# enoche/MMRec

Hardware: AMD Instinct MI355X
Metric: GCN-layer edges/sec (3-layer user-item CSR SpMM, d=64, fp32) (higher is better)
Workload: dtype f32

## Files before the change

### include/mmrec_hip.h

```cpp
#ifndef MMREC_HIP_H
#define MMREC_HIP_H

#include <stddef.h>
#include <stdint.h>

#ifdef __cplusplus
extern "C" {
#endif

#define MMREC_ABI_VERSION 16
#define MMREC_EMB_DIM 64

#define MMREC_ERR_BAD_ARG 10001
#define MMREC_ERR_UNSUPPORTED 10002

typedef void* mmrec_stream_t;

int mmrec_abi_version(void);
const char* mmrec_error_string(int err);

#ifndef MMREC_SPMM_CHUNK
#define MMREC_SPMM_CHUNK 512
#endif
#define MMREC_SPMM_LONG_ROW_DEFAULT 32

int mmrec_spmm_csr_f32(const int32_t* rowptr, const int32_t* colidx, const float* vals,
                       const float* X, float* Y, const float* Z, const float* acc_in, float* acc_out,
                       int32_t n_rows, int32_t d, float alpha, float beta, float acc_scale,
                       int32_t long_row_threshold, const int32_t* long_rows,
                       const int32_t* long_chunk_ptr, int32_t n_long, int32_t n_chunks,
                       float* partials, int32_t* long_tickets, mmrec_stream_t stream);

int mmrec_spmm_rows_f32(const int32_t* rowptr, const int32_t* colidx, const float* vals, const float* X,
                        const float* Z, int32_t z_compact, const int64_t* rows, int32_t n_list, int32_t d,
                        int32_t long_row_threshold, float* Y, mmrec_stream_t stream);
int mmrec_spmm_rows_any_f32(const int32_t* rowptr, const int32_t* colidx, const float* vals, const float* X,
                            const float* Z, int32_t z_compact, const int64_t* rows, int32_t n_list, int32_t d,
                            int32_t long_row_threshold, int32_t max_row_chunks, float* Y, mmrec_stream_t stream);
int mmrec_spmm_push_rows_f32(const int32_t* rowptr, const int32_t* colidx, const float* vals, const float* G,
                             float g_scale, const int64_t* rows, int32_t n_list, int32_t d, float* dX, float* dZ,
                             mmrec_stream_t stream);

int mmrec_spmm_csr_f32_layergcn(const int32_t* rowptr, const int32_t* colidx, const float* vals, const float* X,
                                float* Y, const float* ego, float* scaled, float* w, const float* acc_in,
                                float* acc_out, int32_t n_rows, int32_t d, int32_t long_row_threshold,
                                const int32_t* long_rows, const int32_t* long_chunk_ptr, int32_t n_long,
                                int32_t n_chunks, float* partials, int32_t* long_tickets, mmrec_stream_t stream);
int mmrec_spmm_plan_count(const int32_t* rowptr_host, int32_t n_rows, int32_t long_row_threshold,
                          int32_t* n_long, int32_t* n_chunks);
int mmrec_spmm_plan_fill(const int32_t* rowptr_host, int32_t n_rows, int32_t long_row_threshold,
                         int32_t* long_rows, int32_t* long_chunk_ptr);

int mmrec_cos_scale_fwd_f32(const float* E, const float* Ego, float* Out, float* w, float* acc,
                            int32_t n_rows, int32_t d, mmrec_stream_t stream);
int mmrec_cos_scale_bwd_f32(const float* dOut, const float* E, const float* Ego, const float* w,
                            float* dE, float* dEgo_accum, int32_t n_rows, int32_t d,
                            mmrec_stream_t stream);

#define MMREC_BPR_LOGSIG 0
#define MMREC_BPR_GAMMA 1

size_t mmrec_bpr_workspace_bytes(int32_t batch);
int mmrec_bpr_fwd_f32(const float* U, const float* P, const float* N, const int64_t* users,
                      const int64_t* pos, const int64_t* neg, int32_t batch, int32_t d,
                      int32_t variant, float scale, float* loss_out, float* coef, void* workspace,
                      mmrec_stream_t stream);
int mmrec_bpr_bwd_f32(const float* U, const float* P, const float* N, const int64_t* users,
                      const int64_t* pos, const int64_t* neg, int32_t batch, int32_t d,
                      const float* coef, const float* grad_scalar, float scale, float* dU, float* dP,
                      float* dN, mmrec_stream_t stream);
// ... 202 lines not shown
```

### mmrec_amd/_lib.py

```python
from __future__ import annotations

import ctypes
import os
from ctypes import c_char_p, c_float, c_int32, c_int64, c_size_t, c_uint64, c_void_p

import torch

_PKG = os.path.dirname(os.path.abspath(__file__))
LIB_PATH = os.environ.get("MMREC_HIP_LIB") or os.path.join(_PKG, "lib", "libmmrec_hip.so")
ABI_VERSION = 16

_P = c_void_p

SIGNATURES = {
    "mmrec_abi_version": (c_int32, []),
    "mmrec_error_string": (c_char_p, [c_int32]),
    "mmrec_spmm_csr_f32": (c_int32, [_P, _P, _P, _P, _P, _P, _P, _P, c_int32, c_int32, c_float,
                                     c_float, c_float, c_int32, _P, _P, c_int32, c_int32, _P, _P, _P]),
    "mmrec_spmm_csr_f32_layergcn": (c_int32, [_P, _P, _P, _P, _P, _P, _P, _P, _P, _P, c_int32, c_int32, c_int32,
                                              _P, _P, c_int32, c_int32, _P, _P, _P]),
    "mmrec_spmm_plan_count": (c_int32, [_P, c_int32, c_int32, _P, _P]),
    "mmrec_spmm_plan_fill": (c_int32, [_P, c_int32, c_int32, _P, _P]),
    "mmrec_cos_scale_fwd_f32": (c_int32, [_P, _P, _P, _P, _P, c_int32, c_int32, _P]),
    "mmrec_cos_scale_bwd_f32": (c_int32, [_P, _P, _P, _P, _P, _P, c_int32, c_int32, _P]),
    "mmrec_bpr_workspace_bytes": (c_size_t, [c_int32]),
    "mmrec_bpr_fwd_f32": (c_int32, [_P, _P, _P, _P, _P, _P, c_int32, c_int32, c_int32, c_float, _P,
                                    _P, _P, _P]),
    "mmrec_spmm_rows_f32": (c_int32, [_P, _P, _P, _P, _P, c_int32, _P, c_int32, c_int32, c_int32, _P, _P]),
    "mmrec_spmm_rows_any_f32": (c_int32, [_P, _P, _P, _P, _P, c_int32, _P, c_int32, c_int32, c_int32, c_int32, _P, _P]),
    "mmrec_spmm_push_rows_f32": (c_int32, [_P, _P, _P, _P, c_float, _P, c_int32, c_int32, _P, _P, _P]),
    "mmrec_bpr_dots_f32": (c_int32, [_P, _P, _P, _P, _P, _P, c_int32, c_int32, _P, _P]),
    "mmrec_bpr_loss_from_dots_f32": (c_int32, [_P, c_int32, c_int32, c_float, _P, _P, _P, _P]),
    "mmrec_bpr_bwd_f32": (c_int32, [_P, _P, _P, _P, _P, _P, c_int32, c_int32, _P, _P, c_float, _P, _P,
                                    _P, _P]),
    "mmrec_gather_sqnorm_fwd_f32": (c_int32, [_P, _P, c_int32, c_int32, _P, _P, _P]),
    "mmrec_gather_scale_add_bwd_f32": (c_int32, [_P, _P, c_int32, c_int32, _P, _P, _P]),
    "mmrec_infonce_workspace_bytes": (c_size_t, [c_int32]),
    "mmrec_infonce_fwd_f32": (c_int32, [_P, _P, _P, c_int32, c_int32, c_float, _P, _P, _P]),
    "mmrec_infonce_bwd_f32": (c_int32, [_P, c_int32, c_int32, c_float, _P, _P, _P, _P, _P]),
    "mmrec_linear_workspace_bytes": (c_size_t, [c_int32, c_int32, c_int32]),
    "mmrec_linear_fwd_f32": (c_int32, [_P, _P, _P, _P, c_int32, c_int32, c_int32, _P, _P]),
    "mmrec_linear_fwd_split_f32": (c_int32, [_P, _P, _P, _P, c_int32, c_int32, c_int32, _P, _P]),
    "mmrec_linear_bwd_split_workspace_bytes": (c_size_t, [c_int32, c_int32, c_int32]),
# ... 107 lines not shown
```

### mmrec_amd/csrc/spmm.hip

```cpp
#include "common.h"
#include "spmm_narrow.h"

#ifndef MMREC_SPMM_RPG
#define MMREC_SPMM_RPG(n_rows) ((n_rows) <= (1 << 18) ? 1 : 4)
#endif

namespace {

__device__ __forceinline__ void st_coherent(float4* p, float4 v) {
    unsigned long long* q = reinterpret_cast<unsigned long long*>(p);
    const unsigned long long lo = ((unsigned long long)__float_as_uint(v.y) << 32) | __float_as_uint(v.x);
    const unsigned long long hi = ((unsigned long long)__float_as_uint(v.w) << 32) | __float_as_uint(v.z);
    __hip_atomic_store(q, lo, __ATOMIC_RELAXED, __HIP_MEMORY_SCOPE_AGENT);
    __hip_atomic_store(q + 1, hi, __ATOMIC_RELAXED, __HIP_MEMORY_SCOPE_AGENT);
}
__device__ __forceinline__ float4 ld_coherent(const float4* p) {
    unsigned long long* q = reinterpret_cast<unsigned long long*>(const_cast<float4*>(p));
    const unsigned long long lo = __hip_atomic_load(q, __ATOMIC_RELAXED, __HIP_MEMORY_SCOPE_AGENT);
    const unsigned long long hi = __hip_atomic_load(q + 1, __ATOMIC_RELAXED, __HIP_MEMORY_SCOPE_AGENT);
    return make_float4(__uint_as_float((unsigned)lo), __uint_as_float((unsigned)(lo >> 32)),
                       __uint_as_float((unsigned)hi), __uint_as_float((unsigned)(hi >> 32)));
}

struct RowEpilogue {
    const float* Z;
    float* Y;
    const float* acc_in;
    float* acc_out;
    float alpha, beta, acc_scale;
    const float* ego;
    float* scaled;
    float* w_out;
};

template <int DCH, bool LG>
__device__ __forceinline__ void store_row(const RowEpilogue& ep, int row, int lane16, const float4 (&sum)[DCH]) {
    if (DCH == 1 && LG) {
        const size_t off = (size_t)row * 16 + lane16;
        const float4 y = f4_scale(ep.alpha, sum[0]);
        const float4 g = reinterpret_cast<const float4*>(ep.ego)[off];
        const float dot = row16_sum(f4_dot(y, g));
        const float ne = fmaxf(sqrtf(row16_sum(f4_dot(y, y))), 1e-8f);
        const float ng = fmaxf(sqrtf(row16_sum(f4_dot(g, g))), 1e-8f);
        const float w = dot / (ne * ng);
        const float4 o = f4_scale(w, y);
        if (ep.Y) reinterpret_cast<float4*>(ep.Y)[off] = y;
        reinterpret_cast<float4*>(ep.scaled)[off] = o;
        if (lane16 == 0) ep.w_out[row] = w;
        if (ep.acc_out)
            reinterpret_cast<float4*>(ep.acc_out)[off] =
                ep.acc_in ? f4_add(reinterpret_cast<const float4*>(ep.acc_in)[off], o) : o;
        return;
    }
#pragma unroll
    for (int ch = 0; ch < DCH; ++ch) {
// ... 49 lines not shown
    const int lane16 = threadIdx.x & 15, g = threadIdx.x >> 4;
#pragma unroll
    for (int ch = 0; ch < DCH; ++ch) {
        float4 t = f4_zero();
        for (int c = c0 + g; c < c1; c += 16) {
            const float4* src = reinterpret_cast<const float4*>(partials) + (size_t)c * (16 * DCH) + ch * 16 + lane16;
            t = f4_add(t, COHERENT ? ld_coherent(src) : *src);
        }
        red[g][ch * 16 + lane16] = t;
    }
    __syncthreads();
    if (g == 0) {
        float4 r[DCH];
#pragma unroll
        for (int ch = 0; ch < DCH; ++ch) {
            r[ch] = red[0][ch * 16 + lane16];
#pragma unroll
            for (int k = 1; k < 16; ++k) r[ch] = f4_add(r[ch], red[k][ch * 16 + lane16]);
        }
        store_row<DCH, LG>(ep, row, lane16, r);
    }
}

template <int DCH, bool LG>
__global__ __launch_bounds__(256) void spmm_rows_kernel(
    const int32_t* __restrict__ rowptr, const int32_t* __restrict__ colidx,
    const float* __restrict__ vals, const float* __restrict__ X, RowEpilogue ep, int n_rows,
    int long_t, int rows_per_group, const int32_t* __restrict__ long_rows,
    const int32_t* __restrict__ long_chunk_ptr, int n_long, int n_chunks,
    float* __restrict__ partials, int32_t* __restrict__ tickets) {
    __shared__ float4 red[16][16 * DCH];
    __shared__ int s_last;
    const int lane16 = threadIdx.x & 15;
    const int g = threadIdx.x >> 4;
    const float4* X4 = reinterpret_cast<const float4*>(X);
    if ((int)blockIdx.x < n_chunks) {
        const int chunk = blockIdx.x;
        int lo = 0, hi = n_long;
        while (hi - lo > 1) {
            const int mid = (lo + hi) >> 1;
            if (long_chunk_ptr[mid] <= chunk) lo = mid; else hi = mid;
        }
        const int row = long_rows[lo];
        const int cs = rowptr[row] + (chunk - long_chunk_ptr[lo]) * MMREC_SPMM_CHUNK;
        const int ce = min(cs + MMREC_SPMM_CHUNK, rowptr[row + 1]);
        float4 acc[DCH];
#pragma unroll
        for (int ch = 0; ch < DCH; ++ch) acc[ch] = f4_zero();
        for (int base = cs + g * 16; base < ce; base += 256)
            gather_span<DCH>(colidx, vals, X4, base, min(base + 16, ce), lane16, acc);
#pragma unroll
        for (int ch = 0; ch < DCH; ++ch) red[g][ch * 16 + lane16] = acc[ch];
        __syncthreads();
// ... 12 lines not shown
                for (int ch = 0; ch < DCH; ++ch) {
                    float4* dst = reinterpret_cast<float4*>(partials) + (size_t)chunk * (16 * DCH) + ch * 16 + lane16;
                    if (tickets) st_coherent(dst, t[ch]); else *dst = t[ch];
                }
            }
        }
        const int c0 = long_chunk_ptr[lo], c1 = long_chunk_ptr[lo + 1];
        if (!tickets || c1 - c0 == 1) return;
        if (threadIdx.x < 64) {
            __atomic_signal_fence(__ATOMIC_SEQ_CST);
            __builtin_amdgcn_s_waitcnt(0);
            __atomic_signal_fence(__ATOMIC_SEQ_CST);
            __builtin_amdgcn_fence(__ATOMIC_RELEASE, "workgroup");
            if (threadIdx.x == 0)
                s_last = __hip_atomic_fetch_add(tickets + lo, 1, __ATOMIC_RELAXED, __HIP_MEMORY_SCOPE_AGENT) == c1 - c0 - 1;
        }
        __syncthreads();
        if (!s_last) return;
        __builtin_amdgcn_fence(__ATOMIC_ACQUIRE, "workgroup");
        reduce_long_row<DCH, true, LG>(partials, c0, c1, row, ep, red);
        if (threadIdx.x == 0) __hip_atomic_store(tickets + lo, 0, __ATOMIC_RELAXED, __HIP_MEMORY_SCOPE_AGENT);
        return;
    }
    const int row0 = ((int)blockIdx.x - n_chunks) * 16 * rows_per_group + g;
#pragma unroll 1
    for (int i = 0; i < rows_per_group; ++i) {
        const int row = row0 + i * 16;
        if (row >= n_rows) break;
        const int s = rowptr[row], e = rowptr[row + 1];
        if (e - s > long_t) continue;
        float4 acc[DCH];
#pragma unroll
        for (int ch = 0; ch < DCH; ++ch) acc[ch] = f4_zero();
        gather_span<DCH>(colidx, vals, X4, s, e, lane16, acc);
        store_row<DCH, LG>(ep, row, lane16, acc);
    }
}

template <int DCH, bool LG>
__global__ __launch_bounds__(256) void spmm_long_reduce_kernel(
    const int32_t* __restrict__ long_rows, const int32_t* __restrict__ long_chunk_ptr, int n_long,
    const float* __restrict__ partials, RowEpilogue ep) {
    __shared__ float4 red[16][16 * DCH];
    const int i = blockIdx.x;
    const int c0 = long_chunk_ptr[i], c1 = long_chunk_ptr[i + 1];
    if (c1 - c0 <= 1) return;
    reduce_long_row<DCH, false, LG>(partials, c0, c1, long_rows[i], ep, red);
}

template <int DCH, bool LG = false>
void launch_spmm(hipStream_t s, int blocks, int nch, const int32_t* rowptr, const int32_t* colidx,
                 const float* vals, const float* X, const RowEpilogue& ep, int n_rows, int long_t,
                 int rows_per_group, const int32_t* long_rows, const int32_t* long_chunk_ptr, int n_long,
                 float* partials, int32_t* tickets) {
    hipLaunchKernelGGL((spmm_rows_kernel<DCH, LG>), dim3(blocks + nch), dim3(256), 0, s, rowptr, colidx, vals, X,
                       ep, n_rows, long_t, rows_per_group, long_rows, long_chunk_ptr, n_long, nch, partials, tickets);
    if (!tickets && n_long > 0 && nch > n_long)
        hipLaunchKernelGGL((spmm_long_reduce_kernel<DCH, LG>), dim3(n_long), dim3(256), 0, s, long_rows,
                           long_chunk_ptr, n_long, partials, ep);
}

__global__ __launch_bounds__(256) void cos_scale_fwd_kernel(const float* __restrict__ E,
                                                            const float* __restrict__ Ego,
                                                            float* __restrict__ Out,
                                                            float* __restrict__ W,
                                                            float* __restrict__ acc, int n_rows) {
    const int lane16 = threadIdx.x & 15;
    const int row = blockIdx.x * 16 + (threadIdx.x >> 4);
    if (row >= n_rows) return;
    const size_t off = (size_t)row * 16 + lane16;
    const float4 e = reinterpret_cast<const float4*>(E)[off];
    const float4 g = reinterpret_cast<const float4*>(Ego)[off];
    const float dot = row16_sum(f4_dot(e, g));
    const float ne = fmaxf(sqrtf(row16_sum(f4_dot(e, e))), 1e-8f);
    const float ng = fmaxf(sqrtf(row16_sum(f4_dot(g, g))), 1e-8f);
    const float w = dot / (ne * ng);
    const float4 o = f4_scale(w, e);
    reinterpret_cast<float4*>(Out)[off] = o;
    if (lane16 == 0) W[row] = w;
// ... 8 lines not shown
    if (row >= n_rows) return;
    const size_t off = (size_t)row * 16 + lane16;
    const float4 e = reinterpret_cast<const float4*>(E)[off];
    const float4 g = reinterpret_cast<const float4*>(Ego)[off];
    const float4 d = reinterpret_cast<const float4*>(dOut)[off];
    const float w = W[row];
    const float ne_raw = sqrtf(row16_sum(f4_dot(e, e)));
    const float ng_raw = sqrtf(row16_sum(f4_dot(g, g)));
    const float ne = fmaxf(ne_raw, 1e-8f), ng = fmaxf(ng_raw, 1e-8f);
    const float dw = row16_sum(f4_dot(d, e));
    const float inv = 1.0f / (ne * ng);
    const float ce = (ne_raw > 1e-8f) ? w / (ne * ne) : 0.f;
    const float cg = (ng_raw > 1e-8f) ? w / (ng * ng) : 0.f;
    float4 de = f4_scale(w, d);
    de = f4_fma(dw * inv, g, de);
    de = f4_fma(-dw * ce, e, de);
    reinterpret_cast<float4*>(dE)[off] = de;
    float4 dg = reinterpret_cast<float4*>(dEgo)[off];
    dg = f4_fma(dw * inv, e, dg);
    dg = f4_fma(-dw * cg, g, dg);
    reinterpret_cast<float4*>(dEgo)[off] = dg;
}

}

extern "C" int mmrec_spmm_csr_f32(const int32_t* rowptr, const int32_t* colidx, const float* vals,
                                  const float* X, float* Y, const float* Z, const float* acc_in,
                                  float* acc_out, int32_t n_rows, int32_t d, float alpha, float beta,
                                  float acc_scale, int32_t long_row_threshold,
                                  const int32_t* long_rows, const int32_t* long_chunk_ptr,
                                  int32_t n_long, int32_t n_chunks, float* partials, int32_t* long_tickets,
                                  mmrec_stream_t stream) {
    const bool narrow = d == 8 || d == 16 || d == 32;
    if (!narrow && (d <= 0 || d % MMREC_EMB_DIM || d / MMREC_EMB_DIM > 6)) return MMREC_ERR_UNSUPPORTED;
    if (n_rows < 0 || n_long < 0 || n_chunks < 0 || long_row_threshold < 0) return MMREC_ERR_BAD_ARG;
    if (n_rows == 0) return 0;
    if (!rowptr || !X || (!Y && !acc_out)) return MMREC_ERR_BAD_ARG;
    if (acc_out && !acc_in) return MMREC_ERR_BAD_ARG;
    if (n_long > 0 && (!long_rows || !long_chunk_ptr || !partials || n_chunks <= 0))
        return MMREC_ERR_BAD_ARG;
    if (Y == X || acc_out == X) return MMREC_ERR_BAD_ARG;
    if (narrow)
        return spmm_narrow_launch(rowptr, colidx, vals, X, Y, Z, acc_in, acc_out, n_rows, d, alpha, beta, acc_scale,
                                  n_long > 0 ? long_row_threshold : INT32_MAX, long_rows, long_chunk_ptr, n_long,
                                  n_long > 0 ? n_chunks : 0, partials, mmrec_stream(stream));
    RowEpilogue ep{Z, Y, acc_in, acc_out, alpha, Z ? beta : 0.f, acc_scale, nullptr, nullptr, nullptr};
// ... 51 lines not shown
                                           const float* X, float* Y, const float* ego, float* scaled, float* w,
                                           const float* acc_in, float* acc_out, int32_t n_rows, int32_t d,
                                           int32_t long_row_threshold, const int32_t* long_rows,
                                           const int32_t* long_chunk_ptr, int32_t n_long, int32_t n_chunks,
                                           float* partials, int32_t* long_tickets, mmrec_stream_t stream) {
    if (d != MMREC_EMB_DIM) return MMREC_ERR_UNSUPPORTED;
    if (n_rows < 0 || n_long < 0 || n_chunks < 0 || long_row_threshold < 0) return MMREC_ERR_BAD_ARG;
    if (n_rows == 0) return 0;
    if (!rowptr || !X || !ego || !scaled || !w) return MMREC_ERR_BAD_ARG;
    if (n_long > 0 && (!long_rows || !long_chunk_ptr || !partials || n_chunks <= 0)) return MMREC_ERR_BAD_ARG;
    if (Y == X || scaled == X || acc_out == X) return MMREC_ERR_BAD_ARG;
    RowEpilogue ep{nullptr, Y, acc_in, acc_out, 1.f, 0.f, 1.f, ego, scaled, w};
    hipStream_t s = mmrec_stream(stream);
    const int rows_per_group = MMREC_SPMM_RPG(n_rows);
    const int blocks = (n_rows + 16 * rows_per_group - 1) / (16 * rows_per_group);
    const int long_t = n_long > 0 ? long_row_threshold : INT32_MAX;
    const int nch = n_long > 0 ? n_chunks : 0;
    int32_t* tickets = n_long > 0 ? long_tickets : nullptr;
    launch_spmm<1, true>(s, blocks, nch, rowptr, colidx, vals, X, ep, n_rows, long_t, rows_per_group, long_rows,
                         long_chunk_ptr, n_long, partials, tickets);
    MMREC_RETURN_LAUNCH_STATUS();
}

extern "C" int mmrec_spmm_plan_count(const int32_t* rowptr_host, int32_t n_rows,
                                     int32_t long_row_threshold, int32_t* n_long, int32_t* n_chunks) {
    if (!rowptr_host || !n_long || !n_chunks || n_rows < 0) return MMREC_ERR_BAD_ARG;
    int32_t nl = 0, nc = 0;
    for (int32_t r = 0; r < n_rows; ++r) {
        const int32_t deg = rowptr_host[r + 1] - rowptr_host[r];
        if (deg > long_row_threshold) {
            ++nl;
            nc += (deg + MMREC_SPMM_CHUNK - 1) / MMREC_SPMM_CHUNK;
        }
    }
    *n_long = nl;
    *n_chunks = nc;
    return 0;
}

extern "C" int mmrec_spmm_plan_fill(const int32_t* rowptr_host, int32_t n_rows,
                                    int32_t long_row_threshold, int32_t* long_rows,
                                    int32_t* long_chunk_ptr) {
    if (!rowptr_host || !long_rows || !long_chunk_ptr || n_rows < 0) return MMREC_ERR_BAD_ARG;
    int32_t nl = 0, nc = 0;
    for (int32_t r = 0; r < n_rows; ++r) {
        const int32_t deg = rowptr_host[r + 1] - rowptr_host[r];
// ... 33 lines not shown
```

### mmrec_amd/hip_ops.py

```python
from __future__ import annotations

import ctypes

import numpy as np
import torch

from . import _lib

EMB_DIM = 64
LINEAR_F16X3_DEFAULT = True
LINEAR_F16X3 = LINEAR_F16X3_DEFAULT
SLICE_WIDTHS = (8, 16, 32)
SPMM_CHUNK = 512
LONG_ROW_DEFAULT = None


def default_long_row_threshold(n_cols):
    import os
    forced = os.environ.get("MMREC_LONG_ROW_THRESHOLD")
    if forced:
        return int(forced)
    return 16 if n_cols <= (1 << 18) else 32

TOPK_MAX = 128
BPR_LOGSIG, BPR_GAMMA = 0, 1

DETERMINISTIC_DEFAULT = False
DETERMINISTIC = DETERMINISTIC_DEFAULT
_TORCH_DET_BY_US = False


def set_deterministic(flag=True):
    global DETERMINISTIC, _TORCH_DET_BY_US
    DETERMINISTIC = bool(flag)
    if DETERMINISTIC and not torch.are_deterministic_algorithms_enabled():
        torch.use_deterministic_algorithms(True, warn_only=True)
        _TORCH_DET_BY_US = True
    elif not DETERMINISTIC and _TORCH_DET_BY_US:
        torch.use_deterministic_algorithms(False)
        _TORCH_DET_BY_US = False


def scatter_add_rows(ids, rows, out):
    lib = _lib.load()
    _chk(ids, torch.int64, "ids", 1)
# ... 11 lines not shown
def _stream():
    return ctypes.c_void_p(torch.cuda.current_stream().cuda_stream)


def _chk(t, dtype, name, dim=None):
    if not isinstance(t, torch.Tensor) or not t.is_cuda:
        raise _lib.MMRecHipError("%s must be a device tensor (the hot path has no CPU fallback)" % name)
    if t.dtype != dtype:
        raise _lib.MMRecHipError("%s must be %s, got %s" % (name, dtype, t.dtype))
    if not t.is_contiguous():
        raise _lib.MMRecHipError("%s must be contiguous" % name)
    if dim is not None and t.dim() != dim:
        raise _lib.MMRecHipError("%s must be %d-d" % (name, dim))
    return t


def _ws(nbytes, device):
    return torch.empty(max(int(nbytes), 16), dtype=torch.uint8, device=device)


class CsrGraph:

    def __init__(self, rowptr, colidx, vals, n_rows, n_cols, symmetric=False,
                 long_row_threshold=LONG_ROW_DEFAULT, rowptr_host=None):
        self.rowptr = _chk(rowptr, torch.int32, "rowptr", 1)
        self.colidx = _chk(colidx, torch.int32, "colidx", 1)
        self.vals = _chk(vals, torch.float32, "vals", 1)
        self.n_rows, self.n_cols = int(n_rows), int(n_cols)
        self.nnz = int(colidx.numel())
        self.symmetric = bool(symmetric)
        self.long_row_threshold = int(default_long_row_threshold(self.n_cols) if long_row_threshold is None
                                      else long_row_threshold)
        self._t = self if symmetric else None
        self._plan(rowptr_host)

    def _plan(self, rowptr_host):
        lib = _lib.load()
        rp = rowptr_host if rowptr_host is not None else self.rowptr.cpu().numpy()
        rp = np.ascontiguousarray(rp, dtype=np.int32)
        self.rowptr_host = rp
        n_long, n_chunks = ctypes.c_int32(0), ctypes.c_int32(0)
        _lib.check(lib.mmrec_spmm_plan_count(rp.ctypes.data_as(ctypes.c_void_p), self.n_rows,
                                             self.long_row_threshold, ctypes.byref(n_long),
                                             ctypes.byref(n_chunks)), "spmm_plan_count")
        self.n_long, self.n_chunks = n_long.value, n_chunks.value
        dev = self.rowptr.device
        if self.n_long > 0:
            lr = np.empty(self.n_long, dtype=np.int32)
            cp = np.empty(self.n_long + 1, dtype=np.int32)
            _lib.check(lib.mmrec_spmm_plan_fill(rp.ctypes.data_as(ctypes.c_void_p), self.n_rows,
                                                self.long_row_threshold,
                                                lr.ctypes.data_as(ctypes.c_void_p),
                                                cp.ctypes.data_as(ctypes.c_void_p)), "spmm_plan_fill")
            self.long_rows = torch.from_numpy(lr).to(dev)
            self.long_chunk_ptr = torch.from_numpy(cp).to(dev)
            self.max_row_chunks = int(np.diff(cp).max())
            self.long_tickets = torch.zeros(self.n_long, dtype=torch.int32, device=dev)
        else:
            self.long_rows = self.long_chunk_ptr = self.long_tickets = None
            self.max_row_chunks = 1
        self._partials = {}

    def checked(self, rc, what):
        try:
            _lib.check(rc, what)
        except _lib.MMRecHipError:
            if self.long_tickets is not None:
                try:
                    self.long_tickets.zero_()
                except RuntimeError:
                    pass
            raise

    def partials_for(self, d):
        if self.n_long == 0:
            return None
        if d not in self._partials:
            self._partials[d] = torch.empty(self.n_chunks * d, dtype=torch.float32, device=self.rowptr.device)
        return self._partials[d]

    @classmethod
    def from_coo_host(cls, idx, val, n_rows, n_cols, device, symmetric=False, **kw):
        idx = np.asarray(idx, dtype=np.int64)
        val = np.asarray(val, dtype=np.float32)
# ... 21 lines not shown
        return cls(rowptr, colidx, vout, n_rows, n_cols, symmetric=symmetric, **kw)

    def to_coo_host(self):
        rp = self.rowptr_host.astype(np.int64)
        rows = np.repeat(np.arange(self.n_rows, dtype=np.int64), np.diff(rp))
        return np.stack([rows, self.colidx.cpu().numpy().astype(np.int64)]), self.vals.cpu().numpy()

    def transpose(self):
        if self._t is None:
            idx, val = self.to_coo_host()
            self._t = CsrGraph.from_coo_host(idx[::-1], val, self.n_cols, self.n_rows,
                                             self.rowptr.device,
                                             long_row_threshold=self.long_row_threshold)
            self._t._t = self
        return self._t

    def row_block(self, r0, r1):
        rp = self.rowptr_host.astype(np.int64)
        s, e = int(rp[r0]), int(rp[r1])
        rph = (rp[r0:r1 + 1] - s).astype(np.int32)
        dev = self.rowptr.device
        return CsrGraph(torch.from_numpy(rph).to(dev), self.colidx[s:e].contiguous(),
                        self.vals[s:e].contiguous(), r1 - r0, self.n_cols,
                        long_row_threshold=self.long_row_threshold, rowptr_host=rph)


def _mode_labels(rows, lab_c, n_rows, n_labels):
    key = rows.astype(np.int64) * n_labels + lab_c
    key.sort()
    start = np.flatnonzero(np.concatenate([[True], key[1:] != key[:-1]]))
    cnt = np.diff(np.concatenate([start, [key.shape[0]]]))
    k = key[start]
    r, lab = k // n_labels, k % n_labels
    o = np.lexsort((lab, -cnt, r))
    r_s = r[o]
    first = np.concatenate([[True], r_s[1:] != r_s[:-1]])
    out = np.full(n_rows, -1, dtype=np.int64)
    out[r_s[first]] = lab[o][first]
    return out


def _mode_labels_device(rows, lab_c, n_rows, n_labels):
    key, _ = torch.sort(rows * n_labels + lab_c)
    uk, cnt = torch.unique_consecutive(key, return_counts=True)
    r, lab = torch.div(uk, n_labels, rounding_mode='floor'), uk % n_labels
    cmax = int(cnt.max().item()) + 1
    if n_rows * cmax * n_labels >= 2 ** 62:
# ... 64 lines not shown
        self.n_rows = self.n_cols = n
        self.nnz = g.nnz

    def to_new(self, X):
        return X.index_select(0, self.inv)

    def to_old(self, Xp):
        return Xp.index_select(0, self.perm)


def spmm_raw(g: CsrGraph, X, Y=None, Z=None, acc_in=None, acc_out=None, alpha=1.0, beta=1.0,
             acc_scale=1.0):
    lib = _lib.load()
    _chk(X, torch.float32, "X", 2)
    d = X.shape[1]
    if (d not in SLICE_WIDTHS and (d % EMB_DIM or d > 6 * EMB_DIM)) or X.shape[0] < g.n_cols:
        raise _lib.MMRecHipError("X must be [>=%d, 64*k <= 384 (or a feature slice of 8 / 16 / 32 columns)], got %s" %
                                 (g.n_cols, tuple(X.shape)))
    for t, nm in ((Y, "Y"), (Z, "Z"), (acc_in, "acc_in"), (acc_out, "acc_out")):
        if t is not None:
            _chk(t, torch.float32, nm, 2)
            if t.shape[0] < g.n_rows or t.shape[1] != d:
                raise _lib.MMRecHipError("%s must be [>=%d, %d]" % (nm, g.n_rows, d))
    g.checked(lib.mmrec_spmm_csr_f32(_p(g.rowptr), _p(g.colidx), _p(g.vals), _p(X), _p(Y), _p(Z),
                                     _p(acc_in), _p(acc_out), g.n_rows, d, float(alpha),
                                     float(beta), float(acc_scale), g.long_row_threshold,
                                     _p(g.long_rows), _p(g.long_chunk_ptr), g.n_long, g.n_chunks,
                                     _p(g.partials_for(d)), _p(g.long_tickets), _stream()), "spmm_csr_f32")
    return Y if Y is not None else acc_out


ROWS_MAX_CHUNKS = 480


def rows_servable(g: CsrGraph, d):
    if d not in SLICE_WIDTHS + (EMB_DIM,):
        return False
    return g.n_chunks == g.n_long or (d == EMB_DIM and g.max_row_chunks <= ROWS_MAX_CHUNKS)


def spmm_rows_raw(g: CsrGraph, X, rows, Z=None, z_compact=False):
    lib = _lib.load()
    _chk(X, torch.float32, "X", 2), _chk(rows, torch.int64, "rows", 1)
    d = X.shape[1]
    if not rows_servable(g, d) or X.shape[0] < g.n_cols:
        raise _lib.MMRecHipError("spmm_rows: graph with multi-chunk rows, or X not [>=%d, 8 / 16 / 32 / 64]" % g.n_cols)
# ... 259 lines not shown

def lightgcn_mean_parts_rows(g: CsrGraph, parts, n_layers, rows):
    if DETERMINISTIC or isinstance(g, PermutedGraph) or parts[0].shape[1] not in SLICE_WIDTHS + (EMB_DIM,):
        return torch.cat(lightgcn_mean_parts(g, parts, n_layers), dim=0).index_select(0, rows)
    return _LightGCNMeanPartsRows.apply(g, n_layers, rows, *parts)


class _LayerGCNSum(torch.autograd.Function):

    @staticmethod
    def forward(ctx, E0, g, n_layers):
        lib = _lib.load()
        E0 = E0.contiguous()
        L, n = int(n_layers), E0.shape[0]
        if E0.shape[1] != EMB_DIM or E0.shape[0] != g.n_rows or g.n_cols != g.n_rows:
            raise _lib.MMRecHipError("layergcn_sum needs E0 [n, %d] over a square graph of n rows" % EMB_DIM)
        acc = torch.zeros_like(E0) if L == 0 else torch.empty_like(E0)
        need_y = any(ctx.needs_input_grad)
        ys, ws = [], []
        cur = E0
        for layer in range(L):
            y = torch.empty_like(E0) if need_y else None
            out, w = torch.empty_like(E0), torch.empty(n, dtype=torch.float32, device=E0.device)
            g.checked(lib.mmrec_spmm_csr_f32_layergcn(
                _p(g.rowptr), _p(g.colidx), _p(g.vals), _p(cur), _p(y), _p(E0), _p(out), _p(w),
                _p(acc) if layer > 0 else None, _p(acc), g.n_rows, EMB_DIM, g.long_row_threshold, _p(g.long_rows),
                _p(g.long_chunk_ptr), g.n_long, g.n_chunks, _p(g.partials_for(EMB_DIM)), _p(g.long_tickets), _stream()),
                "spmm_layergcn")
            ys.append(y), ws.append(w)
            cur = out
        ctx.g, ctx.L = g, L
        if need_y:
            ctx.save_for_backward(E0, *ys, *ws)
        return acc

    @staticmethod
    def backward(ctx, dSum):
        lib = _lib.load()
        L, gt = ctx.L, ctx.g.transpose()
        saved = ctx.saved_tensors
        E0, ys, ws = saved[0], saved[1:1 + L], saved[1 + L:]
        dSum = dSum.contiguous()
        n = E0.shape[0]
        dEgo = torch.zeros_like(E0)
        dOut = dSum
        for layer in range(L - 1, -1, -1):
            dY = torch.empty_like(E0)
            _lib.check(lib.mmrec_cos_scale_bwd_f32(_p(dOut), _p(ys[layer]), _p(E0), _p(ws[layer]),
                                                   _p(dY), _p(dEgo), n, EMB_DIM, _stream()),
                       "cos_scale_bwd")
            nxt = torch.empty_like(E0)
# ... 877 lines not shown
    rows = torch.empty(2 * E, dtype=torch.int32, device=dev)
    cols = torch.empty(2 * E, dtype=torch.int32, device=dev)
    vals = torch.empty(2 * E, dtype=torch.float32, device=dev)
    _lib.check(lib.mmrec_bipartite_expand(_p(eu), _p(ei), _p(w), E, n_users, _p(rows), _p(cols),
                                          _p(vals), _stream()), "bipartite_expand")
    n = n_users + n_items
    return CsrGraph.from_coo_device(rows, cols, vals, n, n, symmetric=True,
                                    long_row_threshold=long_row_threshold)


class DynGraph:

    def __init__(self, rows, cols, n_rows, n_cols, long_row_threshold=LONG_ROW_DEFAULT):
        _chk(rows, torch.int64, "rows", 1), _chk(cols, torch.int64, "cols", 1)
        self.rows, self.cols, self.n_rows, self.n_cols = rows, cols, int(n_rows), int(n_cols)
        dev = rows.device
        zeros = torch.zeros(rows.numel(), dtype=torch.float32, device=dev)

        def build(r, c, nr, nc):
            perm = torch.sort(r, stable=True)[1]
            rowptr = torch.zeros(nr + 1, dtype=torch.int64, device=dev)
            rowptr[1:] = torch.cumsum(torch.bincount(r, minlength=nr), 0)
            g = CsrGraph(rowptr.to(torch.int32), c[perm].to(torch.int32).contiguous(), zeros, nr, nc,
                         long_row_threshold=long_row_threshold)
            return g, perm
        self.fwd, self.perm = build(rows, cols, self.n_rows, self.n_cols)
        self.bwd, self.perm_t = build(cols, rows, self.n_cols, self.n_rows)


class _SpMMVals(torch.autograd.Function):
    @staticmethod
    def forward(ctx, X, vals, dyn):
        X = X.contiguous()
        dyn.fwd.vals = vals.detach()[dyn.perm].contiguous()
        Y = torch.empty(dyn.n_rows, X.shape[1], dtype=torch.float32, device=X.device)
        spmm_raw(dyn.fwd, X, Y=Y)
        ctx.dyn = dyn
        ctx.save_for_backward(X, vals)
        return Y

    @staticmethod
    def backward(ctx, dY):
        dyn = ctx.dyn
        X, vals = ctx.saved_tensors
        dY = dY.contiguous()
        dX = dvals = None
        if ctx.needs_input_grad[0]:
# ... 310 lines not shown
```

Before: 29.28 billion.

## Reorder short rows by shared high-degree key column for cache locality

Adds a row schedule for large graphs (more than 2^18 columns). Short rows are permuted so that rows sharing the same moderately high-degree neighbour column run close together, and their column and value arrays are copied into a contiguous reordered buffer. The scheduled kernel walks this permuted list, aiming to improve L2 reuse of gathered X rows during SpMM. In exchange it costs extra memory for a second copy of colidx and vals plus a one-time planning pass, and it is only active when the graph exceeds the column threshold.

```diff
diff --git a/include/mmrec_hip.h b/include/mmrec_hip.h
--- a/include/mmrec_hip.h
+++ b/include/mmrec_hip.h
@@ -46,6 +46,22 @@
                                 float* acc_out, int32_t n_rows, int32_t d, int32_t long_row_threshold,
                                 const int32_t* long_rows, const int32_t* long_chunk_ptr, int32_t n_long,
                                 int32_t n_chunks, float* partials, int32_t* long_tickets, mmrec_stream_t stream);
+int mmrec_spmm_csr_sched_f32(const int32_t* rowptr, const int32_t* colidx, const float* vals, const float* X, float* Y,
+                             const float* Z, const float* acc_in, float* acc_out, int32_t n_rows, int32_t d, float alpha,
+                             float beta, float acc_scale, int32_t long_row_threshold, const int32_t* long_rows,
+                             const int32_t* long_chunk_ptr, int32_t n_long, int32_t n_chunks, float* partials,
+                             int32_t* long_tickets, const int32_t* sched_row, const int32_t* sched_span,
+                             const int32_t* sched_col, const float* sched_val, int32_t n_short, mmrec_stream_t stream);
+int mmrec_spmm_csr_sched_f32_layergcn(const int32_t* rowptr, const int32_t* colidx, const float* vals, const float* X,
+                                      float* Y, const float* ego, float* scaled, float* w, const float* acc_in,
+                                      float* acc_out, int32_t n_rows, int32_t d, int32_t long_row_threshold,
+                                      const int32_t* long_rows, const int32_t* long_chunk_ptr, int32_t n_long,
+                                      int32_t n_chunks, float* partials, int32_t* long_tickets, const int32_t* sched_row,
+                                      const int32_t* sched_span, const int32_t* sched_col, const float* sched_val,
+                                      int32_t n_short, mmrec_stream_t stream);
+int mmrec_spmm_row_keys(const int32_t* rowptr, const int32_t* colidx, const int32_t* col_degree, int32_t n_rows,
+                        int32_t long_row_threshold, int32_t key_deg_max, int32_t* key, int32_t* key_degree,
+                        mmrec_stream_t stream);
 int mmrec_spmm_plan_count(const int32_t* rowptr_host, int32_t n_rows, int32_t long_row_threshold,
                           int32_t* n_long, int32_t* n_chunks);
 int mmrec_spmm_plan_fill(const int32_t* rowptr_host, int32_t n_rows, int32_t long_row_threshold,
diff --git a/mmrec_amd/_lib.py b/mmrec_amd/_lib.py
--- a/mmrec_amd/_lib.py
+++ b/mmrec_amd/_lib.py
@@ -19,6 +19,12 @@
                                      c_float, c_float, c_int32, _P, _P, c_int32, c_int32, _P, _P, _P]),
     "mmrec_spmm_csr_f32_layergcn": (c_int32, [_P, _P, _P, _P, _P, _P, _P, _P, _P, _P, c_int32, c_int32, c_int32,
                                               _P, _P, c_int32, c_int32, _P, _P, _P]),
+    "mmrec_spmm_csr_sched_f32": (c_int32, [_P, _P, _P, _P, _P, _P, _P, _P, c_int32, c_int32, c_float,
+                                           c_float, c_float, c_int32, _P, _P, c_int32, c_int32, _P, _P,
+                                           _P, _P, _P, _P, c_int32, _P]),
+    "mmrec_spmm_csr_sched_f32_layergcn": (c_int32, [_P, _P, _P, _P, _P, _P, _P, _P, _P, _P, c_int32, c_int32, c_int32,
+                                                    _P, _P, c_int32, c_int32, _P, _P, _P, _P, _P, _P, c_int32, _P]),
+    "mmrec_spmm_row_keys": (c_int32, [_P, _P, _P, c_int32, c_int32, c_int32, _P, _P, _P]),
     "mmrec_spmm_plan_count": (c_int32, [_P, c_int32, c_int32, _P, _P]),
     "mmrec_spmm_plan_fill": (c_int32, [_P, c_int32, c_int32, _P, _P]),
     "mmrec_cos_scale_fwd_f32": (c_int32, [_P, _P, _P, _P, _P, c_int32, c_int32, _P]),
diff --git a/mmrec_amd/csrc/spmm.hip b/mmrec_amd/csrc/spmm.hip
--- a/mmrec_amd/csrc/spmm.hip
+++ b/mmrec_amd/csrc/spmm.hip
@@ -31,6 +31,14 @@
     const float* ego;
     float* scaled;
     float* w_out;
+};
+
+struct RowSchedule {
+    const int32_t* row;
+    const int2* span;
+    const int32_t* col;
+    const float* val;
+    int n_short;
 };
 
 template <int DCH, bool LG>
@@ -126,13 +134,13 @@
     }
 }
 
-template <int DCH, bool LG>
+template <int DCH, bool LG, bool SCHED>
 __global__ __launch_bounds__(256) void spmm_rows_kernel(
     const int32_t* __restrict__ rowptr, const int32_t* __restrict__ colidx,
     const float* __restrict__ vals, const float* __restrict__ X, RowEpilogue ep, int n_rows,
     int long_t, int rows_per_group, const int32_t* __restrict__ long_rows,
     const int32_t* __restrict__ long_chunk_ptr, int n_long, int n_chunks,
-    float* __restrict__ partials, int32_t* __restrict__ tickets) {
+    float* __restrict__ partials, int32_t* __restrict__ tickets, RowSchedule sched) {
     __shared__ float4 red[16][16 * DCH];
     __shared__ int s_last;
     const int lane16 = threadIdx.x & 15;
@@ -191,6 +199,22 @@
         if (threadIdx.x == 0) __hip_atomic_store(tickets + lo, 0, __ATOMIC_RELAXED, __HIP_MEMORY_SCOPE_AGENT);
         return;
     }
+    if (SCHED) {
+        const int slot0 = ((int)blockIdx.x - n_chunks) * 16 * rows_per_group + g;
+#pragma unroll 1
+        for (int i = 0; i < rows_per_group; ++i) {
+            const int slot = slot0 + i * 16;
+            if (slot >= sched.n_short) break;
+            const int row = sched.row[slot];
+            const int2 se = sched.span[slot];
+            float4 acc[DCH];
+#pragma unroll
+            for (int ch = 0; ch < DCH; ++ch) acc[ch] = f4_zero();
+            gather_span<DCH>(sched.col, sched.val, X4, se.x, se.y, lane16, acc);
+            store_row<DCH, LG>(ep, row, lane16, acc);
+        }
+        return;
+    }
     const int row0 = ((int)blockIdx.x - n_chunks) * 16 * rows_per_group + g;
 #pragma unroll 1
     for (int i = 0; i < rows_per_group; ++i) {
@@ -217,13 +241,15 @@
     reduce_long_row<DCH, false, LG>(partials, c0, c1, long_rows[i], ep, red);
 }
 
-template <int DCH, bool LG = false>
+template <int DCH, bool LG = false, bool SCHED = false>
 void launch_spmm(hipStream_t s, int blocks, int nch, const int32_t* rowptr, const int32_t* colidx,
                  const float* vals, const float* X, const RowEpilogue& ep, int n_rows, int long_t,
                  int rows_per_group, const int32_t* long_rows, const int32_t* long_chunk_ptr, int n_long,
-                 float* partials, int32_t* tickets) {
-    hipLaunchKernelGGL((spmm_rows_kernel<DCH, LG>), dim3(blocks + nch), dim3(256), 0, s, rowptr, colidx, vals, X,
-                       ep, n_rows, long_t, rows_per_group, long_rows, long_chunk_ptr, n_long, nch, partials, tickets);
+                 float* partials, int32_t* tickets, const RowSchedule& sched = RowSchedule{}) {
+    if (blocks + nch > 0)
+        hipLaunchKernelGGL((spmm_rows_kernel<DCH, LG, SCHED>), dim3(blocks + nch), dim3(256), 0, s, rowptr, colidx, vals, X,
+                           ep, n_rows, long_t, rows_per_group, long_rows, long_chunk_ptr, n_long, nch, partials, tickets,
+                           sched);
     if (!tickets && n_long > 0 && nch > n_long)
         hipLaunchKernelGGL((spmm_long_reduce_kernel<DCH, LG>), dim3(n_long), dim3(256), 0, s, long_rows,
                            long_chunk_ptr, n_long, partials, ep);
@@ -278,6 +304,41 @@
     reinterpret_cast<float4*>(dEgo)[off] = dg;
 }
 
+__global__ __launch_bounds__(256) void spmm_row_keys_kernel(const int32_t* __restrict__ rowptr,
+                                                            const int32_t* __restrict__ colidx,
+                                                            const int32_t* __restrict__ col_degree, int n_rows, int long_t,
+                                                            int deg_max, int32_t* __restrict__ key,
+                                                            int32_t* __restrict__ key_degree) {
+    const int lane16 = threadIdx.x & 15;
+    const int row = blockIdx.x * 16 + (threadIdx.x >> 4);
+    if (row >= n_rows) return;
+    const int s = rowptr[row], e = rowptr[row + 1];
+    int bd = 0, bp = INT32_MAX, bc = -1;
+    if (e - s <= long_t)
+        for (int k = s + lane16; k < e; k += 16) {
+            const int c = colidx[k];
+            const int dg = col_degree[c];
+            if (dg <= deg_max && dg > bd) {
+                bd = dg;
+                bp = k;
+                bc = c;
+            }
+        }
+#pragma unroll
+    for (int m = 8; m > 0; m >>= 1) {
+        const int od = __shfl_xor(bd, m, 16), op = __shfl_xor(bp, m, 16), oc = __shfl_xor(bc, m, 16);
+        if (od > bd || (od == bd && op < bp)) {
+            bd = od;
+            bp = op;
+            bc = oc;
+        }
+    }
+    if (lane16 == 0) {
+        key[row] = bc;
+        key_degree[row] = bd;
+    }
+}
+
 }
 
 extern "C" int mmrec_spmm_csr_f32(const int32_t* rowptr, const int32_t* colidx, const float* vals,
@@ -375,6 +436,91 @@
     MMREC_RETURN_LAUNCH_STATUS();
 }
 
+namespace {
+bool sched_args_ok(const int32_t* sched_row, const int32_t* sched_span, const int32_t* sched_col, const float* sched_val,
+                   int32_t n_short, int32_t n_rows) {
+    if (n_short < 0 || n_short > n_rows) return false;
+    return n_short == 0 || (sched_row && sched_span && sched_col && sched_val);
+}
+}
+
+extern "C" int mmrec_spmm_csr_sched_f32(const int32_t* rowptr, const int32_t* colidx, const float* vals,
+                                        const float* X, float* Y, const float* Z, const float* acc_in,
+                                        float* acc_out, int32_t n_rows, int32_t d, float alpha, float beta,
+                                        float acc_scale, int32_t long_row_threshold,
+                                        const int32_t* long_rows, const int32_t* long_chunk_ptr,
+                                        int32_t n_long, int32_t n_chunks, float* partials, int32_t* long_tickets,
+                                        const int32_t* sched_row, const int32_t* sched_span, const int32_t* sched_col,
+                                        const float* sched_val, int32_t n_short, mmrec_stream_t stream) {
+    if (d <= 0 || d % MMREC_EMB_DIM || d / MMREC_EMB_DIM > 6) return MMREC_ERR_UNSUPPORTED;
+    if (n_rows < 0 || n_long < 0 || n_chunks < 0 || long_row_threshold < 0) return MMREC_ERR_BAD_ARG;
+    if (n_rows == 0) return 0;
+    if (!rowptr || !X || (!Y && !acc_out)) return MMREC_ERR_BAD_ARG;
+    if (acc_out && !acc_in) return MMREC_ERR_BAD_ARG;
+    if (n_long > 0 && (!long_rows || !long_chunk_ptr || !partials || n_chunks <= 0))
+        return MMREC_ERR_BAD_ARG;
+    if (!sched_args_ok(sched_row, sched_span, sched_col, sched_val, n_short, n_rows)) return MMREC_ERR_BAD_ARG;
+    if (Y == X || acc_out == X) return MMREC_ERR_BAD_ARG;
+    RowEpilogue ep{Z, Y, acc_in, acc_out, alpha, Z ? beta : 0.f, acc_scale, nullptr, nullptr, nullptr};
+    const RowSchedule sched{sched_row, reinterpret_cast<const int2*>(sched_span), sched_col, sched_val, n_short};
+    hipStream_t s = mmrec_stream(stream);
+    const int rows_per_group = MMREC_SPMM_RPG(n_rows);
+    const int blocks = (n_short + 16 * rows_per_group - 1) / (16 * rows_per_group);
+    const int long_t = n_long > 0 ? long_row_threshold : INT32_MAX;
+    const int nch = n_long > 0 ? n_chunks : 0;
+    int32_t* tickets = n_long > 0 ? long_tickets : nullptr;
+#define MMREC_SPMM_CASE(D)                                                                                      \
+    case D:                                                                                                     \
+        launch_spmm<D, false, true>(s, blocks, nch, rowptr, colidx, vals, X, ep, n_rows, long_t, rows_per_group, \
+                                    long_rows, long_chunk_ptr, n_long, partials, tickets, sched);               \
+        break;
+    switch (d / MMREC_EMB_DIM) {
+        MMREC_SPMM_CASE(1) MMREC_SPMM_CASE(2) MMREC_SPMM_CASE(3) MMREC_SPMM_CASE(4) MMREC_SPMM_CASE(5)
+        MMREC_SPMM_CASE(6)
+    }
+#undef MMREC_SPMM_CASE
+    MMREC_RETURN_LAUNCH_STATUS();
+}
+
+extern "C" int mmrec_spmm_csr_sched_f32_layergcn(const int32_t* rowptr, const int32_t* colidx, const float* vals,
+                                                 const float* X, float* Y, const float* ego, float* scaled, float* w,
+                                                 const float* acc_in, float* acc_out, int32_t n_rows, int32_t d,
+                                                 int32_t long_row_threshold, const int32_t* long_rows,
+                                                 const int32_t* long_chunk_ptr, int32_t n_long, int32_t n_chunks,
+                                                 float* partials, int32_t* long_tickets, const int32_t* sched_row,
+                                                 const int32_t* sched_span, const int32_t* sched_col,
+                                                 const float* sched_val, int32_t n_short, mmrec_stream_t stream) {
+    if (d != MMREC_EMB_DIM) return MMREC_ERR_UNSUPPORTED;
+    if (n_rows < 0 || n_long < 0 || n_chunks < 0 || long_row_threshold < 0) return MMREC_ERR_BAD_ARG;
+    if (n_rows == 0) return 0;
+    if (!rowptr || !X || !ego || !scaled || !w) return MMREC_ERR_BAD_ARG;
+    if (n_long > 0 && (!long_rows || !long_chunk_ptr || !partials || n_chunks <= 0)) return MMREC_ERR_BAD_ARG;
+    if (!sched_args_ok(sched_row, sched_span, sched_col, sched_val, n_short, n_rows)) return MMREC_ERR_BAD_ARG;
+    if (Y == X || scaled == X || acc_out == X) return MMREC_ERR_BAD_ARG;
+    RowEpilogue ep{nullptr, Y, acc_in, acc_out, 1.f, 0.f, 1.f, ego, scaled, w};
+    const RowSchedule sched{sched_row, reinterpret_cast<const int2*>(sched_span), sched_col, sched_val, n_short};
+    hipStream_t s = mmrec_stream(stream);
+    const int rows_per_group = MMREC_SPMM_RPG(n_rows);
+    const int blocks = (n_short + 16 * rows_per_group - 1) / (16 * rows_per_group);
+    const int long_t = n_long > 0 ? long_row_threshold : INT32_MAX;
+    const int nch = n_long > 0 ? n_chunks : 0;
+    int32_t* tickets = n_long > 0 ? long_tickets : nullptr;
+    launch_spmm<1, true, true>(s, blocks, nch, rowptr, colidx, vals, X, ep, n_rows, long_t, rows_per_group, long_rows,
+                               long_chunk_ptr, n_long, partials, tickets, sched);
+    MMREC_RETURN_LAUNCH_STATUS();
+}
+
+extern "C" int mmrec_spmm_row_keys(const int32_t* rowptr, const int32_t* colidx, const int32_t* col_degree,
+                                   int32_t n_rows, int32_t long_row_threshold, int32_t key_deg_max, int32_t* key,
+                                   int32_t* key_degree, mmrec_stream_t stream) {
+    if (n_rows < 0 || long_row_threshold < 0 || key_deg_max < 0) return MMREC_ERR_BAD_ARG;
+    if (n_rows == 0) return 0;
+    if (!rowptr || !colidx || !col_degree || !key || !key_degree) return MMREC_ERR_BAD_ARG;
+    hipLaunchKernelGGL(spmm_row_keys_kernel, dim3((n_rows + 15) / 16), dim3(256), 0, mmrec_stream(stream), rowptr, colidx,
+                       col_degree, n_rows, long_row_threshold, key_deg_max, key, key_degree);
+    MMREC_RETURN_LAUNCH_STATUS();
+}
+
 extern "C" int mmrec_spmm_plan_count(const int32_t* rowptr_host, int32_t n_rows,
                                      int32_t long_row_threshold, int32_t* n_long, int32_t* n_chunks) {
     if (!rowptr_host || !n_long || !n_chunks || n_rows < 0) return MMREC_ERR_BAD_ARG;
diff --git a/mmrec_amd/hip_ops.py b/mmrec_amd/hip_ops.py
--- a/mmrec_amd/hip_ops.py
+++ b/mmrec_amd/hip_ops.py
@@ -21,6 +21,17 @@
     if forced:
         return int(forced)
     return 16 if n_cols <= (1 << 18) else 32
+
+
+ROW_SCHEDULE_MIN_COLS = 1 << 18
+SPMM_KEY_DEG_MAX = 128
+
+
+def spmm_key_deg_max():
+    import os
+    forced = os.environ.get("MMREC_SPMM_KEY_DEG_MAX")
+    return int(forced) if forced else SPMM_KEY_DEG_MAX
+
 
 TOPK_MAX = 128
 BPR_LOGSIG, BPR_GAMMA = 0, 1
@@ -78,7 +89,7 @@
 class CsrGraph:
 
     def __init__(self, rowptr, colidx, vals, n_rows, n_cols, symmetric=False,
-                 long_row_threshold=LONG_ROW_DEFAULT, rowptr_host=None):
+                 long_row_threshold=LONG_ROW_DEFAULT, rowptr_host=None, row_schedule=None):
         self.rowptr = _chk(rowptr, torch.int32, "rowptr", 1)
         self.colidx = _chk(colidx, torch.int32, "colidx", 1)
         self.vals = _chk(vals, torch.float32, "vals", 1)
@@ -88,6 +99,7 @@
         self.long_row_threshold = int(default_long_row_threshold(self.n_cols) if long_row_threshold is None
                                       else long_row_threshold)
         self._t = self if symmetric else None
+        self.row_schedule = bool(self.n_cols > ROW_SCHEDULE_MIN_COLS if row_schedule is None else row_schedule)
         self._plan(rowptr_host)
 
     def _plan(self, rowptr_host):
@@ -116,6 +128,53 @@
             self.long_rows = self.long_chunk_ptr = self.long_tickets = None
             self.max_row_chunks = 1
         self._partials = {}
+        self.sched = None
+        if self.row_schedule:
+            self._plan_schedule()
+
+    def _plan_schedule(self):
+        lib = _lib.load()
+        dev, n = self.rowptr.device, self.n_rows
+        deg = (self.rowptr[1:] - self.rowptr[:-1])
+        short = torch.nonzero(deg <= self.long_row_threshold).squeeze(1)
+        key = torch.full((n,), -1, dtype=torch.int32, device=dev)
+        kdeg = torch.zeros(n, dtype=torch.int32, device=dev)
+        if self.nnz > 0 and n > 0:
+            if self.symmetric and self.n_cols == n:
+                coldeg = deg.contiguous()
+            else:
+                coldeg = torch.bincount(self.colidx, minlength=self.n_cols).to(torch.int32)
+            _lib.check(lib.mmrec_spmm_row_keys(_p(self.rowptr), _p(self.colidx), _p(coldeg), n, self.long_row_threshold,
+                                               spmm_key_deg_max(), _p(key), _p(kdeg), _stream()), "spmm_row_keys")
+        self.row_key, self.row_key_degree = key, kdeg
+        k, kd, dg = key[short].long(), kdeg[short].long(), deg[short].long()
+        first = self.colidx[self.rowptr[:-1][short].long().clamp_(max=max(self.nnz - 1, 0))].long() if self.nnz > 0 else k
+        ref = torch.where(k >= 0, k, torch.where(dg > 0, first, torch.full_like(k, -1)))
+        band = (ref <= short).long()
+        comp = (band << 62) | (((1 << 31) - 1 - kd) << 31) | k.clamp(min=0)
+        order = torch.sort(comp, stable=True)[1]
+        rows = short[order]
+        lens = dg[order]
+        end = torch.cumsum(lens, 0)
+        begin = end - lens
+        total = int(end[-1].item()) if rows.numel() else 0
+        src0 = self.rowptr[:-1].long()[rows]
+        pos = torch.arange(total, dtype=torch.int64, device=dev) + torch.repeat_interleave(src0 - begin, lens, output_size=total)
+        self.sched = {
+            "row": rows.to(torch.int32).contiguous(),
+            "span": torch.stack([begin, end], 1).to(torch.int32).contiguous(),
+            "col": self.colidx.index_select(0, pos) if total else torch.zeros(1, dtype=torch.int32, device=dev),
+            "val": self.vals.index_select(0, pos) if total else torch.zeros(1, dtype=torch.float32, device=dev),
+            "n_short": int(rows.numel()),
+            "vals_of": self.vals,
+        }
+
+    def scheduled(self, d):
+        sc = self.sched
+        return sc if sc is not None and d % EMB_DIM == 0 and sc["vals_of"] is self.vals else None
+
+    def schedule_bytes(self):
+        return 0 if self.sched is None else sum(self.sched[k].numel() * self.sched[k].element_size() for k in ("row", "span", "col", "val"))
 
     def checked(self, rc, what):
         try:
@@ -183,7 +242,7 @@
         dev = self.rowptr.device
         return CsrGraph(torch.from_numpy(rph).to(dev), self.colidx[s:e].contiguous(),
                         self.vals[s:e].contiguous(), r1 - r0, self.n_cols,
-                        long_row_threshold=self.long_row_threshold, rowptr_host=rph)
+                        long_row_threshold=self.long_row_threshold, rowptr_host=rph, row_schedule=self.row_schedule)
 
 
 def _mode_labels(rows, lab_c, n_rows, n_labels):
@@ -294,6 +353,15 @@
             _chk(t, torch.float32, nm, 2)
             if t.shape[0] < g.n_rows or t.shape[1] != d:
                 raise _lib.MMRecHipError("%s must be [>=%d, %d]" % (nm, g.n_rows, d))
+    sc = g.scheduled(d)
+    if sc is not None:
+        g.checked(lib.mmrec_spmm_csr_sched_f32(_p(g.rowptr), _p(g.colidx), _p(g.vals), _p(X), _p(Y), _p(Z),
+                                               _p(acc_in), _p(acc_out), g.n_rows, d, float(alpha),
+                                               float(beta), float(acc_scale), g.long_row_threshold,
+                                               _p(g.long_rows), _p(g.long_chunk_ptr), g.n_long, g.n_chunks,
+                                               _p(g.partials_for(d)), _p(g.long_tickets), _p(sc["row"]), _p(sc["span"]),
+                                               _p(sc["col"]), _p(sc["val"]), sc["n_short"], _stream()), "spmm_csr_sched_f32")
+        return Y if Y is not None else acc_out
     g.checked(lib.mmrec_spmm_csr_f32(_p(g.rowptr), _p(g.colidx), _p(g.vals), _p(X), _p(Y), _p(Z),
                                      _p(acc_in), _p(acc_out), g.n_rows, d, float(alpha),
                                      float(beta), float(acc_scale), g.long_row_threshold,
@@ -599,11 +667,15 @@
         for layer in range(L):
             y = torch.empty_like(E0) if need_y else None
             out, w = torch.empty_like(E0), torch.empty(n, dtype=torch.float32, device=E0.device)
-            g.checked(lib.mmrec_spmm_csr_f32_layergcn(
-                _p(g.rowptr), _p(g.colidx), _p(g.vals), _p(cur), _p(y), _p(E0), _p(out), _p(w),
-                _p(acc) if layer > 0 else None, _p(acc), g.n_rows, EMB_DIM, g.long_row_threshold, _p(g.long_rows),
-                _p(g.long_chunk_ptr), g.n_long, g.n_chunks, _p(g.partials_for(EMB_DIM)), _p(g.long_tickets), _stream()),
-                "spmm_layergcn")
+            args = (_p(g.rowptr), _p(g.colidx), _p(g.vals), _p(cur), _p(y), _p(E0), _p(out), _p(w),
+                    _p(acc) if layer > 0 else None, _p(acc), g.n_rows, EMB_DIM, g.long_row_threshold, _p(g.long_rows),
+                    _p(g.long_chunk_ptr), g.n_long, g.n_chunks, _p(g.partials_for(EMB_DIM)), _p(g.long_tickets))
+            sc = g.scheduled(EMB_DIM)
+            if sc is not None:
+                g.checked(lib.mmrec_spmm_csr_sched_f32_layergcn(*args, _p(sc["row"]), _p(sc["span"]), _p(sc["col"]), _p(sc["val"]),
+                                                                sc["n_short"], _stream()), "spmm_sched_layergcn")
+            else:
+                g.checked(lib.mmrec_spmm_csr_f32_layergcn(*args, _stream()), "spmm_layergcn")
             ys.append(y), ws.append(w)
             cur = out
         ctx.g, ctx.L = g, L
@@ -1527,7 +1599,7 @@
             rowptr = torch.zeros(nr + 1, dtype=torch.int64, device=dev)
             rowptr[1:] = torch.cumsum(torch.bincount(r, minlength=nr), 0)
             g = CsrGraph(rowptr.to(torch.int32), c[perm].to(torch.int32).contiguous(), zeros, nr, nc,
-                         long_row_threshold=long_row_threshold)
+                         long_row_threshold=long_row_threshold, row_schedule=False)
             return g, perm
         self.fwd, self.perm = build(rows, cols, self.n_rows, self.n_cols)
         self.bwd, self.perm_t = build(cols, rows, self.n_cols, self.n_rows)
```

Result: faster. 31.22 billion, median of 6 (+6.6%).
